# penn-graphics-research/claymore

Hardware: AMD Instinct MI355X
Metric: particles*steps/sec (higher is better)
Workload: dtype f32

## Files before the change

### claymore_amd/csrc/claymore_hip.hip

```cpp
#include <hip/hip_runtime.h>

#include <algorithm>
#include <cmath>
#include <cstdio>
#include <cstdlib>
#include <chrono>
#include <cstring>
#include <string>
#include <vector>

#include "../../include/claymore_amd.h"
#include "mpm_kernels.hpp"
#include "mpm_readout.hpp"

using namespace mpm;

namespace {
constexpr int kHaloWords	 = 128;
constexpr int kStatusBlock = ST_WORDS + kHaloWords + kMaxVelSlots * kMaxVelStride;

struct Partition {
	int* table = nullptr;
	int* keys  = nullptr;
	int* count = nullptr;
// ... 545 lines not shown
	if(ctx->nbc) {
		const int est = std::min(ctx->g.cap, ctx->nbc + ctx->nbc / 16 + 64);
		if(ctx->has_collision)
			grid_update_collision_kernel<<<cdiv(est, 4), 256, 0, s>>>(ctx->g, &ctx->d_status[ST_NBC], ctx->grid[0], ctx->part[ctx->rollid].keys, dt, collision_tick(ctx, dt), ctx->d_maxvel);
		else
			grid_update_kernel<<<cdiv(est, 16), 256, 0, s>>>(ctx->g, &ctx->d_status[ST_NBC], ctx->grid[0], ctx->part[ctx->rollid].keys, dt, ctx->d_maxvel);
	}
	return MPM_OK;
}

int mpm_grid_update(mpm_ctx* ctx, float dt, float* max_vel_sqr) {
	phase_call(ctx);
	if(!ctx || !ctx->ready) return MPM_ERR_NOT_READY;
	HIP_TRY(hipSetDevice(ctx->device));
	hipStream_t s = ctx->s_compute;
	HIP_TRY(hipEventRecord(ctx->ev.start, s));
	int rc = launch_grid_update(ctx, dt);
	if(rc) return rc;
	HIP_TRY(hipEventRecord(ctx->ev.end, s));
	HIP_TRY(hipMemcpyAsync(ctx->h_maxvel, ctx->d_maxvel, sizeof(float) * kMaxVelSlots * kMaxVelStride, hipMemcpyDeviceToHost, s));
	HIP_TRY(hipStreamSynchronize(s));
	HIP_TRY(hipEventElapsedTime(&ctx->timers.grid_update_ms, ctx->ev.start, ctx->ev.end));
	if(max_vel_sqr) *max_vel_sqr = host_maxvel(ctx);
	return MPM_OK;
}

float mpm_compute_dt(const mpm_ctx* ctx, float max_vel, float cur_time, float next_time, float dt_default) {
	float dt = dt_default;
	if(max_vel > 0.0f) dt = std::min(ctx->g.dx * ctx->cfg.cfl / max_vel, dt);
	return std::min(dt, next_time - cur_time);
}

static ModelView make_view(mpm_ctx* ctx, Model& m) {
	const int r = ctx->rollid, n = r ^ 1;
	ModelView v {};
	v.bins_src	 = m.bins[r];
	v.bins_dst	 = m.bins[n];
	v.binoff_src = m.binoff[r];
	v.binoff_dst = m.binoff[n];
	v.list_in	 = m.list[m.list_in];
	v.list_out	 = m.list[m.list_in ^ 1];
	v.size		 = m.size;
	v.row_of	 = m.row_of;
	v.out_count	 = m.out_count;
	v.keep		 = m.keep;
	v.blockinfo	 = m.blockinfo;
	v.pairinfo_in  = m.pairinfo[0];
	v.pairinfo_out = m.pairinfo[1];
	v.mc		 = m.mc;
	return v;
}

static ReadoutArgs make_readout_args(mpm_ctx* ctx, const Model& m) {
	const int r = ctx->rollid;
	return ReadoutArgs {ctx->g, m.nch, m.pair ? 1 : 0, ctx->part[r].keys, ctx->part[r].table, ctx->part[r ^ 1].table, m.size, m.row_of, m.list[m.list_in], m.binoff[r], m.bins[r]};
}

static inline int hint_blocks(const mpm_ctx* ctx, int n) {
	const long long h = (long long) n + n / 16 + 64;
	return (int) ((std::min<long long>(h, std::max(ctx->g.cap, 8)) + 7) & ~7ll);
}

static void launch_g2p2g_model(mpm_ctx* ctx, Model& m, const int* block_list, const int* nblocks_ptr, int nblocks, float dt, float next_dt, hipStream_t s, const int* only_flag = nullptr) {
	const int r = ctx->rollid;
	ModelView v = make_view(ctx, m);
	const int* cur_keys	  = ctx->part[r].keys;
	const GridCfg& g = ctx->g;
	StepConst sk;
	sk.dtp	= dt * g.dx_inv;
	sk.dts	= dt * (4.f * g.dx_inv);
	sk.pred = next_dt * g.dx_inv;
	sk.am	= m.mc.mass * g.dx * g.dx * g.d_inv;
	const float cs = -next_dt * g.d_inv * g.dx;
	sk.ss	= StressScale {2.f * m.mc.mu * m.mc.volume * cs, m.mc.lambda * m.mc.volume * cs, m.mc.volume * cs};
	sk.refl_lim = sk.dts > 0.f ? (1.f / 3.f) / sk.dts : 3.0e38f;
	sk.jdiv		= g.dx * dt * g.d_inv;
	sk.jvisc	= g.dx * g.d_inv * m.mc.viscosity;
	const int nwg = nblocks_ptr ? hint_blocks(ctx, nblocks) : nblocks;
	auto kernel = g2p2g_for<3>(m.pair);
	switch(m.material) {
		case MPM_J_FLUID: kernel = g2p2g_for<0>(m.pair); break;
		case MPM_FIXED_COROTATED: kernel = g2p2g_for<1>(m.pair); break;
		case MPM_SAND: kernel = g2p2g_for<2>(m.pair); break;
		default: break;
	}
	kernel<<<nwg, kG2P2GThreads, 0, s>>>(ctx->g, v, cur_keys, ctx->grid[0], ctx->grid[1], block_list, only_flag, nblocks_ptr, nblocks, dt, next_dt, sk, ctx->d_status);
}

static int launch_clear(mpm_ctx* ctx, int flags) {
	if((flags & kClearRebuild) && !(flags & kClearP2G)) {
		if(ctx->rebuild_cleared) flags &= ~(kClearRebuild | kClearMaxVel);
		ctx->rebuild_cleared = false;
	}
	if(!(flags & (kClearP2G | kClearRebuild))) return MPM_OK;
	ClearArgs a {};
	a.flags	  = flags;
	a.nmodels = (int) ctx->models.size();
	for(int mi = 0; mi < a.nmodels; ++mi) a.out_count[mi] = ctx->models[mi].out_count, a.keep[mi] = ctx->models[mi].keep;
	a.p2g_grid	   = ctx->grid[1];
	a.status	   = ctx->d_status;
	a.max_vel_bits = ctx->d_maxvel;
	Partition& Pn  = ctx->part[ctx->rollid ^ 1];
	a.old_table	   = Pn.table;
	a.old_keys	   = Pn.keys;
	a.old_count	   = Pn.count;
	substep_clear_kernel<<<1024, 256, 0, ctx->s_compute>>>(ctx->g, a);
	return MPM_OK;
}
static int launch_g2p2g_prologue(mpm_ctx* ctx, bool with_rebuild = false, bool fused_update = false) {
	int rc = launch_clear(ctx, with_rebuild ? (kClearP2G | kClearRebuild | (fused_update ? kClearMaxVel : 0)) : kClearP2G);
	if(rc == MPM_OK && with_rebuild) ctx->rebuild_cleared = true;
	return rc;
}

static int launch_g2p2g(mpm_ctx* ctx, float dt, float next_dt, hipEvent_t e0, hipEvent_t e1, bool with_rebuild_clear = false, bool fused_update = false) {
	hipStream_t s = ctx->s_compute;
	int rc		  = launch_g2p2g_prologue(ctx, with_rebuild_clear, fused_update);
	if(rc) return rc;
	HIP_TRY(hipEventRecord(e0, s));
	if(ctx->pbc)
		for(auto& m: ctx->models) launch_g2p2g_model(ctx, m, nullptr, &ctx->d_status[ST_PBC], ctx->pbc, dt, next_dt, s);
	HIP_TRY(hipEventRecord(e1, s));
	return MPM_OK;
}

int mpm_g2p2g(mpm_ctx* ctx, float dt, float next_dt) {
	phase_call(ctx);
	if(!ctx || !ctx->ready) return MPM_ERR_NOT_READY;
	HIP_TRY(hipSetDevice(ctx->device));
	int rc = launch_g2p2g(ctx, dt, next_dt, ctx->ev.g2p2g_start, ctx->ev.g2p2g_end);
	if(rc) return rc;
	HIP_TRY(hipGetLastError());
	HIP_TRY(hipStreamSynchronize(ctx->s_compute));
	HIP_TRY(hipEventElapsedTime(&ctx->last_g2p2g_ms, ctx->ev.g2p2g_start, ctx->ev.g2p2g_end));
	ctx->timers.g2p2g_ms = ctx->last_g2p2g_ms;
	return MPM_OK;
}

static int launch_prepare(mpm_ctx* ctx, int cur, int prev, bool list_is_out, int binoff_sel, const int* pbc_ptr, int nblocks_est, bool sort, bool publish) {
	if(nblocks_est <= 0 && !publish) return MPM_OK;
	PrepareModels pm {};
	pm.n = (int) ctx->models.size();
	for(int mi = 0; mi < pm.n; ++mi) {
		Model& m		  = ctx->models[mi];
		pm.list[mi]		  = m.list[list_is_out ? (m.list_in ^ 1) : m.list_in];
		pm.size[mi]		  = m.size;
		pm.row_of[mi]	  = m.row_of;
		pm.binoff_src[mi] = m.binoff[binoff_sel];
		pm.blockinfo[mi]  = m.blockinfo;
		pm.keep[mi]		  = sort && list_is_out ? m.keep : nullptr;
		pm.pairinfo[mi]	  = m.pair ? m.pairinfo[0] : nullptr;
		pm.pairhand[mi]	  = m.pairinfo[1];
	}
	const int nwg = std::max(1, std::min(ctx->g.cap, nblocks_est + nblocks_est / 16 + 64));
	int* pub	  = publish ? ctx->d_status : nullptr;
	if(sort)
		prepare_blocks_kernel<true><<<nwg, 64, 0, ctx->s_compute>>>(ctx->g, pm, pbc_ptr, ctx->part[cur].table, ctx->part[cur].keys, ctx->part[prev].table, pub, ctx->part[cur].count);
	else
		prepare_blocks_kernel<false><<<nwg, 64, 0, ctx->s_compute>>>(ctx->g, pm, pbc_ptr, ctx->part[cur].table, ctx->part[cur].keys, ctx->part[prev].table, pub, ctx->part[cur].count);
	return MPM_OK;
}

static int launch_rebuild_prepare(mpm_ctx* ctx) {
	const int r = ctx->rollid, n = r ^ 1;
	const int ebc_est = std::min(ctx->g.cap, ctx->ebc + ctx->ebc / 16 + 1024);
	return launch_prepare(ctx, n, r, true, n, &ctx->d_status[ST_CNT_P], ebc_est, true, true);
}
static int launch_rebuild(mpm_ctx* ctx, float fuse_dt = 0.f, bool without_prepare = false) {
	if(fuse_dt == 0.f) fuse_dt = ctx->fuse_dt_once;
	ctx->fuse_dt_once = 0.f;
	hipStream_t s = ctx->s_compute;
	GridCfg& g	  = ctx->g;
	const int r = ctx->rollid, n = r ^ 1;
	Partition& Pn = ctx->part[n];
	Partition& Pr = ctx->part[r];
	const bool fused = fuse_dt > 0.f;
	ctx->grid_momentum = !fused;
	int rc			 = launch_clear(ctx, kClearRebuild | (fused ? kClearMaxVel : 0));
	if(rc) return rc;
	RebuildModels rm {};
	rm.n = (int) ctx->models.size();
	for(int mi = 0; mi < rm.n; ++mi) {
		Model& m		 = ctx->models[mi];
		rm.out_count[mi] = m.out_count;
		rm.size[mi]		 = m.size;
		rm.row_of[mi]	 = m.row_of;
		rm.binoff[mi]	 = m.binoff[r];
		rm.bin_cap[mi]	 = (long long) m.bin_cap;
	}
	int* st			  = ctx->d_status;
	const int ebc_est = std::min(g.cap, ctx->ebc + ctx->ebc / 16 + 1024);
	compact_blocks_kernel<<<std::max(1u, cdiv(ebc_est, 1024)), 1024, 0, s>>>(g, rm, Pr.keys, Pn.keys, Pn.table, st);
	const unsigned rg8 = std::max(1u, std::min(4096u, cdiv((size_t) ebc_est * 8, 256))), rg32 = std::max(1u, std::min(8192u, cdiv((size_t) ebc_est * 32, 256)));
	register_blocks_kernel<0, 1><<<rg8, 256, 0, s>>>(g, &st[ST_CNT_P], nullptr, &st[ST_CNT_N], &st[ST_PBC], Pn.table, Pn.keys, st);
	if(fused) {
		if(ctx->has_collision)
			carry_grid_kernel<true, true><<<2048, 256, 0, s>>>(g, st, Pn.keys, Pr.table, ctx->grid[1], ctx->grid[0], fuse_dt, ctx->d_maxvel, collision_tick(ctx, fuse_dt));
		else
			carry_grid_kernel<true><<<2048, 256, 0, s>>>(g, st, Pn.keys, Pr.table, ctx->grid[1], ctx->grid[0], fuse_dt, ctx->d_maxvel, NoCollision {});
		ctx->grid_preupdated = true;
		ctx->preupdate_dt	 = fuse_dt;
	} else
		carry_grid_kernel<false><<<2048, 256, 0, s>>>(g, st, Pn.keys, Pr.table, ctx->grid[1], ctx->grid[0], 0.f, nullptr, NoCollision {});
	register_blocks_kernel<-1, 1><<<rg32, 256, 0, s>>>(g, &st[ST_CNT_P], &st[ST_CNT_N], &st[ST_CNT_E], &st[ST_NBC], Pn.table, Pn.keys, st);
	if(without_prepare) return MPM_OK;
	return launch_prepare(ctx, n, r, true, n, &st[ST_CNT_P], ebc_est, true, true);
}

static int grow_capacity(mpm_ctx* ctx) {
	if(!ctx->cfg.grow) return MPM_OK;
	hipStream_t s	   = ctx->s_compute;
	const size_t table = (size_t) ctx->g.G * ctx->g.G * ctx->g.G;
	const size_t cap   = (size_t) ctx->g.cap;
	if((size_t) ctx->ebc * 4 > cap * 3 && cap < table) {
		const size_t ncap = std::min(table, cap * 3 / 2 + 1);
		HIP_TRY(hipDeviceSynchronize());
		for(int i = 0; i < 2; ++i) {
			HIP_TRY(regrow(&ctx->part[i].keys, 3 * cap, 3 * ncap, s));
			HIP_TRY(regrow(&ctx->grid[i], cap * 256, ncap * 256, s));
		}
		for(auto& m: ctx->models) {
			for(int i = 0; i < 2; ++i) {
				HIP_TRY(regrow(&m.binoff[i], cap + 1, ncap + 1, s));
				HIP_TRY(regrow(&m.list[i], cap * (size_t) ctx->g.ppb, ncap * (size_t) ctx->g.ppb, s));
			}
			HIP_TRY(regrow(&m.size, cap + 1, ncap + 1, s));
			HIP_TRY(regrow(&m.row_of, cap + 1, ncap + 1, s));
			HIP_TRY(regrow(&m.out_count, cap + 1, ncap + 1, s));
			HIP_TRY(regrow(&m.keep, cap + 1, ncap + 1, s));
			HIP_TRY(regrow(&m.blockinfo, cap * (size_t) kInfoRow, ncap * (size_t) kInfoRow, s));
			if(m.pair)
				for(int i = 0; i < 2; ++i) HIP_TRY(regrow(&m.pairinfo[i], (cap + 1) * (size_t) kPairChunks, (ncap + 1) * (size_t) kPairChunks, s));
		}
		if(ctx->d_overlap) {
			HIP_TRY(regrow(&ctx->d_overlap, cap + 1, ncap + 1, s));
			HIP_TRY(regrow(&ctx->d_halo_list, cap + 1, ncap + 1, s));
			HIP_TRY(regrow(&ctx->d_inner_list, cap + 1, ncap + 1, s));
		}
		for(int p = 0; p < 32; ++p)
			if(ctx->d_send_ids[p]) HIP_TRY(regrow(&ctx->d_send_ids[p], cap + 1, ncap + 1, s));
		ctx->g.cap = (int) ncap;
		ctx->capacity_events++;
	}
	for(auto& m: ctx->models) {
		const size_t need = m.n / kBin + (size_t) ctx->g.cap + 1;
		if((size_t) m.bincount * 4 > m.bin_cap * 3 || need > m.bin_cap) {
			const size_t nb = std::max(need, (size_t) m.bincount * 4 > m.bin_cap * 3 ? m.bin_cap * 3 / 2 + 1 : m.bin_cap);
			HIP_TRY(hipDeviceSynchronize());
			for(int i = 0; i < 2; ++i) HIP_TRY(regrow(&m.bins[i], m.bin_cap * m.nch * kBin, nb * m.nch * kBin, s));
			m.bin_cap = nb;
			ctx->capacity_events++;
		}
	}
	return MPM_OK;
}

static void roll_partition(mpm_ctx* ctx) {
	for(auto& m: ctx->models) m.list_in ^= 1;
	ctx->rollid ^= 1;
}

static int check_books(mpm_ctx* ctx) {
	const long long gone = (long long) ctx->h_status[ST_LOST] + (long long) ctx->h_status[ST_DROPPED] + ctx->books_bias;
	long long added = 0, held = 0;
	for(size_t mi = 0; mi < ctx->models.size(); ++mi) {
		const Model& m = ctx->models[mi];
		added += (long long) m.n;
		held += (long long) m.bucketed;
		if(gone == 0 && (long long) m.bucketed != (long long) m.n)
			return fail(ctx, MPM_ERR_INTERNAL,
						"particle books of model " + std::to_string(mi) + " do not balance: " + std::to_string(m.bucketed) + " bucketed of " + std::to_string(m.n) +
							" added, none counted as lost or dropped");
	}
	if(held + gone != added)
		return fail(ctx, MPM_ERR_INTERNAL,
					"particle books do not balance: " + std::to_string(held) + " bucketed + " + std::to_string(ctx->h_status[ST_LOST]) + " lost + " + std::to_string(ctx->h_status[ST_DROPPED]) +
						" dropped != " + std::to_string(added) + " added");
	return MPM_OK;
}

static int apply_status(mpm_ctx* ctx, mpm_counts* counts);
static int sync_counts(mpm_ctx* ctx, mpm_counts* counts) {
	int rc = read_status(ctx);
	if(rc) return rc;
	return apply_status(ctx, counts);
}
static int apply_status(mpm_ctx* ctx, mpm_counts* counts) {
	int rc = check_status(ctx);
	if(rc) return rc;
	ctx->pbc = ctx->h_status[ST_PBC];
	ctx->nbc = ctx->h_status[ST_NBC];
	ctx->ebc = ctx->h_status[ST_EBC];
	ctx->pbc_prev = ctx->h_status[ST_PBCPREV];
	if(ctx->ebc > ctx->g.cap) return fail(ctx, MPM_ERR_CAPACITY, "Too much exterior blocks: " + std::to_string(ctx->ebc));
	for(size_t mi = 0; mi < ctx->models.size(); ++mi) {
		Model& m	   = ctx->models[mi];
		m.bincount_src = ctx->h_status[ST_BINSPREV + mi];
		m.bincount	   = ctx->h_status[ST_BINS0 + mi];
		m.bucketed	   = ctx->h_status[ST_PART0 + mi];
		if((size_t) m.bincount > m.bin_cap) return fail(ctx, MPM_ERR_CAPACITY, "bin capacity exceeded");
	}
	if(ctx->h_status[ST_NONFINITE]) return fail(ctx, MPM_ERR_NONFINITE, "Maximum velocity is infinity");
	rc = check_books(ctx);
	if(rc) return rc;
	rc = grow_capacity(ctx);
	if(rc) return rc;
	if(counts) return mpm_get_counts(ctx, counts);
// ... 427 lines not shown
```

### claymore_amd/csrc/mpm_kernels.hpp

```cpp
#pragma once
#include <hip/hip_runtime.h>
#include <type_traits>

#include "mpm_device_math.hpp"
#include "mpm_collision.hpp"

namespace mpm {

constexpr int kBin		  = 64;
constexpr int kG2P2GThreads = 64;
constexpr int kMaxModels  = 8;
constexpr int kSortKeys		= 216;
constexpr int kKeyBits		= 8;
constexpr int kStay		  = 13;

enum {
	ST_PBC = 0, ST_NBC = 1, ST_EBC = 2, ST_OVERFLOW = 3, ST_LOST = 4, ST_ARENA = 5, ST_DROPPED = 6, ST_NONFINITE = 7, ST_BINS0 = 8, ST_PART0 = 16,
	 ST_CNT_P = 29, ST_CNT_N = 30, ST_CNT_E = 31, ST_BINSPREV = 32, ST_PBCPREV = 40, ST_WORDS = 64
};

struct GridCfg {
	int G;
	int gbits;
	int ppb;
// ... 154 lines not shown
		const float4 m = g[0];
		float4 p0 = g[16], p1 = g[32], p2 = g[48];
		const float gdt = cfg.gravity * dt;
#define MPM_CELL(c)                                                                 \
	if(m.c > 0.0f) {                                                                \
		const float mass_inv = 1.f / m.c;                                           \
		const float v0		 = wx ? 0.0f : p0.c * mass_inv;                         \
		const float v1		 = (wy ? 0.0f : p1.c * mass_inv) + gdt;                 \
		const float v2		 = wz ? 0.0f : p2.c * mass_inv;                         \
		p0.c				 = v0;                                                  \
		p1.c				 = v1;                                                  \
		p2.c				 = v2;                                                  \
		float q				 = v0 * v0 + v1 * v1 + v2 * v2;                         \
		if(q != q) q = __builtin_inff();  \
		vel_sqr = fmaxf(vel_sqr, q);                                                \
	}
		MPM_CELL(x)
		MPM_CELL(y)
		MPM_CELL(z)
		MPM_CELL(w)
#undef MPM_CELL
		g[16] = p0;
		g[32] = p1;
		g[48] = p2;
	}
#pragma unroll
	for(int off = 32; off > 0; off >>= 1) vel_sqr = fmaxf(vel_sqr, __shfl_xor(vel_sqr, off));
	if((threadIdx.x & 63) == 0 && vel_sqr > 0.f) {
		const unsigned bits = __float_as_uint(vel_sqr);
		unsigned* slot		= max_vel_bits + (blockIdx.x & (kMaxVelSlots - 1)) * kMaxVelStride;
		if(bits > __hip_atomic_load(slot, __ATOMIC_RELAXED, __HIP_MEMORY_SCOPE_AGENT)) atomicMax(slot, bits);
	}
}

struct CollisionArgs {
	CollisionObject obj;
	CollisionPose pose;
};
struct NoCollision {};
MPM_DEV float grid_cell_collision(const GridCfg& cfg, const CollisionArgs& col, int kx, int ky, int kz, int cell, float dt, float4& v) {
#pragma clang fp contract(off)
	const bool wx = kx < cfg.boundary || kx >= cfg.G - cfg.boundary;
	const bool wy = ky < cfg.boundary || ky >= cfg.G - cfg.boundary;
	const bool wz = kz < cfg.boundary || kz >= cfg.G - cfg.boundary;
	const float mass_inv = 1.f / v.x;
	float vel[3];
	vel[0] = wx ? 0.0f : v.y * mass_inv;
	vel[1] = (wy ? 0.0f : v.z * mass_inv) + cfg.gravity * dt;
	vel[2] = wz ? 0.0f : v.w * mass_inv;
	const int node[3] = {kx * 4 + (cell >> 4), ky * 4 + ((cell >> 2) & 3), kz * 4 + (cell & 3)};
	collision_resolve(col.obj, col.pose, node, cfg.dx, cfg.G * 4, (float) cfg.boundary * cfg.dx * 4.f, (float) (cfg.G - cfg.boundary) * 4.f * cfg.dx, vel);
	v.y		= vel[0];
	v.z		= vel[1];
	v.w		= vel[2];
	float q = vel[0] * vel[0] + vel[1] * vel[1] + vel[2] * vel[2];
	q += vel[0] * vel[0];
	q += vel[1] * vel[1];
	q += vel[2] * vel[2];
	if(q != q) q = __builtin_inff();
	return q;
}
__global__ __launch_bounds__(256) void grid_update_collision_kernel(GridCfg cfg, const int* __restrict__ nbc_ptr, float* __restrict__ grid, const int* __restrict__ keys, float dt, CollisionArgs col, unsigned* __restrict__ max_vel_bits) {
	const int cell	  = threadIdx.x & 63;
	const int nblocks = min(*nbc_ptr, cfg.cap);
	float vel_sqr	  = 0.f;
	for(int blockno = (blockIdx.x * 256 + threadIdx.x) >> 6; blockno < nblocks; blockno += gridDim.x * 4) {
		const int kx = keys[3 * blockno], ky = keys[3 * blockno + 1], kz = keys[3 * blockno + 2];
		float* g	 = grid + (size_t) blockno * 256 + cell;
		float4 v	 = {g[0], 0.f, 0.f, 0.f};
		if(v.x > 0.0f) {
			v.y = g[64];
			v.z = g[128];
			v.w = g[192];
			vel_sqr = fmaxf(vel_sqr, grid_cell_collision(cfg, col, kx, ky, kz, cell, dt, v));
			g[64]	= v.y;
			g[128]	= v.z;
			g[192]	= v.w;
		}
	}
#pragma unroll
	for(int off = 32; off > 0; off >>= 1) vel_sqr = fmaxf(vel_sqr, __shfl_xor(vel_sqr, off));
	if((threadIdx.x & 63) == 0 && vel_sqr > 0.f) {
		const unsigned bits = __float_as_uint(vel_sqr);
		unsigned* slot		= max_vel_bits + (blockIdx.x & (kMaxVelSlots - 1)) * kMaxVelStride;
		if(bits > __hip_atomic_load(slot, __ATOMIC_RELAXED, __HIP_MEMORY_SCOPE_AGENT)) atomicMax(slot, bits);
	}
}

__global__ __launch_bounds__(64) void pack_lists_kernel(int ppb, const int* __restrict__ size, const int* __restrict__ row_of, const long long* __restrict__ offset, const int* __restrict__ list, int* __restrict__ packed, int dense, const int* __restrict__ pairinfo, int* __restrict__ packed_info) {
	const int b = blockIdx.x;
	const int n = size[b];
	const int* row = list + (size_t) row_of[b] * ppb;
	for(int i = threadIdx.x; i < n; i += 64) {
		const int chunk = i / kListChunk;
		packed[offset[b] + i] = dense ? row[i] : row[chunk * kListChunk + chunk_slot(chunk_records(n, chunk), i - chunk * kListChunk)];
	}
	if(dense && threadIdx.x < kPairChunks) packed_info[(size_t) b * kPairChunks + threadIdx.x] = pairinfo[(size_t) b * kPairChunks + threadIdx.x];
}
__global__ __launch_bounds__(64) void unpack_lists_kernel(int ppb, const int* __restrict__ size, int* __restrict__ row_of, const long long* __restrict__ offset, int* __restrict__ list, const int* __restrict__ packed, int dense, int* __restrict__ pairinfo, const int* __restrict__ packed_info) {
	const int b = blockIdx.x;
	const int n = size[b];
	int* row	= list + (size_t) b * ppb;
	for(int i = threadIdx.x; i < n; i += 64) {
		const int chunk = i / kListChunk;
		if(dense)
			row[i] = packed[offset[b] + i];
		else
			row[chunk * kListChunk + chunk_slot(chunk_records(n, chunk), i - chunk * kListChunk)] = packed[offset[b] + i];
	}
	if(dense && threadIdx.x < kPairChunks) pairinfo[(size_t) b * kPairChunks + threadIdx.x] = packed_info[(size_t) b * kPairChunks + threadIdx.x];
	if(threadIdx.x == 0) row_of[b] = b;
}
__global__ __launch_bounds__(256) void table_from_keys_kernel(GridCfg cfg, int n, const int* __restrict__ keys, int* __restrict__ table) {
	const int i = blockIdx.x * 256 + threadIdx.x;
	if(i < n) table[key_index(cfg, keys[3 * i], keys[3 * i + 1], keys[3 * i + 2])] = i;
}

__global__ __launch_bounds__(256) void pack_sdf_kernel(size_t n, const float* __restrict__ sd, const float* __restrict__ gx, const float* __restrict__ gy, const float* __restrict__ gz, float4* __restrict__ out) {
	const size_t i = (size_t) blockIdx.x * 256 + threadIdx.x;
	if(i < n) out[i] = make_float4(sd[i], gx[i], gy[i], gz[i]);
}

__device__ __forceinline__ void dir_components(int dir, int& dx, int& dy, int& dz) {
	dz = (dir % 3) - 1;
	dy = ((dir / 3) % 3) - 1;
	dx = (dir / 9) - 1;
}

constexpr int kInfoRow = 64;
struct PrepareModels {
	int n;
	int* list[kMaxModels];
	const int* size[kMaxModels];
	const int* row_of[kMaxModels];
	const int* binoff_src[kMaxModels];
	int* blockinfo[kMaxModels];
	const int* keep[kMaxModels];
	int* pairinfo[kMaxModels];
	const int* pairhand[kMaxModels];
};
template<bool SORT>
__global__ __launch_bounds__(64) void prepare_blocks_kernel(GridCfg cfg, PrepareModels pm, const int* __restrict__ pbc_ptr, const int* __restrict__ cur_table, const int* __restrict__ cur_keys, const int* __restrict__ prev_table, int* __restrict__ publish, int* __restrict__ part_count) {
	constexpr int kPrepChunk = kListChunk;
	__shared__ int s_sorted[kPairChunkMax];
	__shared__ int s_cnt[256];
	__shared__ int s_cur[256];
	const int lane = threadIdx.x;
	if(publish && blockIdx.x == 0 && lane == 0) {
		const int ebc	 = publish[ST_CNT_P] + publish[ST_CNT_N] + publish[ST_CNT_E];
		publish[ST_EBC] = ebc;
		*part_count		 = ebc;
	}
	const int pbc = min(*pbc_ptr, cfg.cap);
	for(int b = blockIdx.x; b < pbc; b += gridDim.x) {
	const int kx = cur_keys[3 * b], ky = cur_keys[3 * b + 1], kz = cur_keys[3 * b + 2];
	int size0 = 0, row0 = 0, keep0 = -2, hand0 = 0;
	if constexpr(SORT) {
		if(pm.n > 0) {
			size0 = pm.size[0][b];
			row0  = pm.row_of[0][b];
			if(pm.keep[0]) keep0 = pm.keep[0][row0];
			if(pm.pairinfo[0]) hand0 = pm.pairhand[0][(size_t) row0 * kPairChunks + (lane & (kPairChunks - 1))];
		}
	}
	int srcno = -1, other = -1;
	if(lane < 27) {
		int ox, oy, oz;
		dir_components(lane, ox, oy, oz);
		srcno = table_query(cfg, prev_table, kx + ox, ky + oy, kz + oz);
	} else if(lane < 54) {
		int ox, oy, oz;
		dir_components(lane - 27, ox, oy, oz);
		other = table_query(cfg, cur_table, kx - ox, ky - oy, kz - oz);
	} else if(lane < 62) {
		const int lb = lane - 54;
		other		 = table_query(cfg, cur_table, kx + ((lb >> 2) & 1), ky + ((lb >> 1) & 1), kz + (lb & 1));
	}
	const int key_shift		= cfg.pid_bits;
	const int tag_shift		= cfg.pid_bits + kKeyBits;
	const unsigned rec_mask = (1u << (tag_shift + 5)) - 1u;
	for(int m = 0; m < pm.n; ++m) {
		int info = other;
		if constexpr(SORT) {
		const int size = __builtin_amdgcn_readfirstlane(m == 0 ? size0 : pm.size[m][b]);
		const int row  = __builtin_amdgcn_readfirstlane(m == 0 ? row0 : pm.row_of[m][b]);
		int* list	   = pm.list[m] + (size_t) row * cfg.ppb;
		const int tail	= size & (kPrepChunk - 1);
		int* pairinfo	= pm.pairinfo[m] ? pm.pairinfo[m] + (size_t) b * kPairChunks : nullptr;
		const int kept	= m == 0 ? keep0 : (pm.keep[m] ? pm.keep[m][row] : -2);
		const bool same = pm.keep[m] && size > 0 && kept == size && (pairinfo || tail <= 64 || (tail & 63) == 0);
		constexpr int NIT = kPrepChunk / 64;
		unsigned recs[NIT];
		auto load_chunk = [&](int chunk0, int nrec) {
#pragma unroll
			for(int it = 0; it < NIT; ++it) recs[it] = (unsigned) list[chunk0 + min(it * 64 + lane, nrec - 1)];
		};
		if(size > 0 && !same) load_chunk(0, min(kPrepChunk, size));
		if(lane < 27) info = srcno >= 0 ? pm.binoff_src[m][srcno] : -1;
		auto sort_chunk = [&](int chunk0, int nrec) {
#pragma unroll
			for(int q = 0; q < 4; ++q) s_cnt[lane + 64 * q] = 0;
			__syncthreads();
			int rank[NIT];
#pragma unroll
			for(int it = 0; it < NIT; ++it) {
				rank[it] = 0;
				if(it * 64 + lane < nrec) rank[it] = atomicAdd(&s_cnt[(recs[it] >> key_shift) & 255], 1);
			}
			__syncthreads();
			{
				const int c0 = s_cnt[4 * lane], c1 = s_cnt[4 * lane + 1], c2 = s_cnt[4 * lane + 2], c3 = s_cnt[4 * lane + 3];
				const int incl = wave_scan_incl(c0 + c1 + c2 + c3);
				const int excl = incl - (c0 + c1 + c2 + c3);
				__syncthreads();
				s_cnt[4 * lane]		= excl;
				s_cnt[4 * lane + 1] = excl + c0;
				s_cnt[4 * lane + 2] = excl + c0 + c1;
				s_cnt[4 * lane + 3] = excl + c0 + c1 + c2;
			}
			__syncthreads();
			const int S = (nrec + 63) >> 6;
			int first[NIT];
#pragma unroll
			for(int it = 0; it < NIT; ++it) first[it] = s_cnt[(recs[it] >> key_shift) & 255];
			__builtin_amdgcn_sched_barrier(0);
#pragma unroll
			for(int it = 0; it < NIT; ++it) {
				if(it * 64 + lane < nrec) {
					const unsigned rec = recs[it] & rec_mask;
					const int p		   = first[it] + rank[it];
					const int pos	   = div_small(p, S);
					s_sorted[(p - pos * S) * 64 + pos] = (int) rec;
				}
			}
			__syncthreads();
			int out[NIT];
#pragma unroll
			for(int it = 0; it < NIT; ++it) out[it] = s_sorted[it * 64 + lane];
			__builtin_amdgcn_sched_barrier(0);
#pragma unroll
			for(int it = 0; it < NIT; ++it)
				if(it < S && lane < slice_records(nrec, it)) list[chunk0 + it * 64 + lane] = out[it];
			__syncthreads();
		};
		auto sort_chunk_pairs = [&](int chunk0, int nrec) {
			const bool big = nrec > kPrepChunk;
			const int n0 = min(nrec, kPrepChunk), n1g = nrec - n0;
#pragma unroll
			for(int q = 0; q < 4; ++q) s_cnt[lane + 64 * q] = 0, s_cur[lane + 64 * q] = 0;
			__syncthreads();
			int rank[NIT];
#pragma unroll
			for(int it = 0; it < NIT; ++it) {
				rank[it] = 0;
				if(it * 64 + lane < n0) rank[it] = atomicAdd(&s_cnt[(recs[it] >> key_shift) & 255], 1);
			}
			if(big) {
#pragma unroll
				for(int it = 0; it < kPairTailMerge / 64; ++it) recs[it] = (unsigned) list[chunk0 + kPrepChunk + min(it * 64 + lane, n1g - 1)];
#pragma unroll
				for(int it = 0; it < kPairTailMerge / 64; ++it)
					if(it * 64 + lane < n1g) atomicAdd(&s_cnt[(recs[it] >> key_shift) & 255], 1);
			}
			__syncthreads();
			int pf;
			{
				int c[4], v[4];
#pragma unroll
				for(int i = 0; i < 4; ++i) {
					c[i] = s_cnt[4 * lane + i];
					v[i] = (c[i] >> 1) | ((c[i] & 1) << 16);
				}
				const int incl = wave_scan_incl(v[0] + v[1] + v[2] + v[3]);
				const int tot  = __builtin_amdgcn_readlane(incl, 63);
				pf			  = tot & 0xffff;
				int excl	  = incl - (v[0] + v[1] + v[2] + v[3]);
#pragma unroll
				for(int i = 0; i < 4; ++i) {
					s_cnt[4 * lane + i] = (excl & 0x3ff) | ((excl >> 16) << 10) | (c[i] << 18);
					excl += v[i];
				}
			}
			__syncthreads();
			const PairChunk pc = pair_chunk(nrec, pf);
			const int n1s	   = pc.L - pc.px;
			auto place = [&](unsigned rec_raw, int r, int e) {
				unsigned rec = rec_raw & rec_mask;
				const int nk = e >> 18, pp = e & 0x3ff;
				int p, member;
				const bool paired = r < (nk & ~1);
				if(paired) {
					p	   = pp + (r >> 1);
					member = r & 1;
				} else {
					const int j = (e >> 10) & 0xff;
					if(j < n1s) {
						p	   = pc.px + j;
						member = 0;
					} else {
						p	   = pc.pf + ((j - n1s) >> 1);
						member = (j - n1s) & 1;
					}
				}
				const int ln = div_small(p, pc.S), d = p - ln * pc.S;
				int pos, ca, cb;
				pair_slice(pc, d, pos, ca, cb);
				int arena = ln & 1;
				if(!paired) {
					int i0 = d - (pp - div_small(pp, pc.S) * pc.S);
					i0 += i0 < 0 ? pc.S : 0;
					if(i0 < (nk >> 1)) arena = 1 ^ (div_small(pp + i0, pc.S) & 1);
				}
				rec |= (unsigned) arena << kArenaBit;
				s_sorted[pos + (member ? ca : 0) + ln] = (int) rec;
			};
			int ent[NIT];
			if(!big) {
#pragma unroll
				for(int it = 0; it < NIT; ++it) ent[it] = s_cnt[(recs[it] >> key_shift) & 255];
				__builtin_amdgcn_sched_barrier(0);
#pragma unroll
				for(int it = 0; it < NIT; ++it)
					if(it * 64 + lane < n0) place(recs[it], rank[it], ent[it]);
			} else {
				auto place_group = [&](int ng) {
#pragma unroll
					for(int it = 0; it < NIT; ++it) {
						if(it * 64 + lane < ng) {
							const int key = (recs[it] >> key_shift) & 255;
							const int r	  = atomicAdd(&s_cur[key], 1);
							place(recs[it], r, s_cnt[key]);
						}
					}
				};
				place_group(n1g);
				load_chunk(chunk0, n0);
				place_group(n0);
			}
			__syncthreads();
			{
				int out[NIT];
#pragma unroll
				for(int it = 0; it < NIT; ++it) out[it] = s_sorted[it * 64 + lane];
				__builtin_amdgcn_sched_barrier(0);
#pragma unroll
				for(int it = 0; it < NIT; ++it)
					if(it * 64 + lane < n0) list[chunk0 + it * 64 + lane] = out[it];
			}
			if(big) {
#pragma unroll
				for(int it = 0; it < kPairTailMerge / 64; ++it)
					if(it * 64 + lane < n1g) list[chunk0 + kPrepChunk + it * 64 + lane] = s_sorted[kPrepChunk + it * 64 + lane];
			}
			if(lane == 0) pairinfo[chunk0 / kPrepChunk] = pf;
			__syncthreads();
		};
		if(pairinfo && same && lane < kPairChunks) pairinfo[lane] = m == 0 ? hand0 : pm.pairhand[m][(size_t) row * kPairChunks + lane];
		for(int chunk0 = 0; chunk0 < size && !same; chunk0 += kPrepChunk) {
			const int left = size - chunk0;
			const int nrec = (pairinfo && left > kPrepChunk && left <= kPairChunkMax) ? left : min(kPrepChunk, left);
			if(chunk0) load_chunk(chunk0, min(kPrepChunk, nrec));
			if(pairinfo)
				sort_chunk_pairs(chunk0, nrec);
			else
				sort_chunk(chunk0, nrec);
			if(nrec > kPrepChunk) break;
		}
		}
		if constexpr(!SORT) {
			if(lane < 27) info = srcno >= 0 ? pm.binoff_src[m][srcno] : -1;
		}
		pm.blockinfo[m][(size_t) b * kInfoRow + lane] = info;
	}
	}
}

}
#include "mpm_g2p2g.hpp"
#include "mpm_g2p2g_pair.hpp"
namespace mpm {

struct RebuildModels {
	int n;
	const int* out_count[kMaxModels];
	int* size[kMaxModels];
	int* row_of[kMaxModels];
	int* binoff[kMaxModels];
	long long bin_cap[kMaxModels];
};

enum { kClearP2G = 1, kClearRebuild = 2, kClearMaxVel = 4 };
struct ClearArgs {
	int flags;
	int nmodels;
	int* out_count[kMaxModels];
	int* keep[kMaxModels];
	float* p2g_grid;
	int* status;
	unsigned* max_vel_bits;
	int* old_table;
	const int* old_keys;
	const int* old_count;
};
__global__ __launch_bounds__(256) void substep_clear_kernel(GridCfg cfg, ClearArgs a) {
	const int tid = blockIdx.x * 256 + threadIdx.x, nthreads = gridDim.x * 256;
	if(a.flags & kClearP2G) {
		const int nbc = min(a.status[ST_NBC], cfg.cap), ebc = min(a.status[ST_EBC], cfg.cap);
		float4* g	  = reinterpret_cast<float4*>(a.p2g_grid);
		for(int i = tid; i < nbc * 64; i += nthreads) g[i] = make_float4(0.f, 0.f, 0.f, 0.f);
		for(int m = 0; m < a.nmodels; ++m)
			for(int i = tid; i <= ebc; i += nthreads) a.out_count[m][i] = 0, a.keep[m][i] = -1;
	}
	if(a.flags & kClearRebuild) {
		const int n = min(*a.old_count, cfg.cap);
		for(int i = tid; i < n; i += nthreads) a.old_table[key_index(cfg, a.old_keys[3 * i], a.old_keys[3 * i + 1], a.old_keys[3 * i + 2])] = -1;
		if(blockIdx.x == gridDim.x - 1) {
			if(threadIdx.x < kMaxModels) {
				a.status[ST_BINSPREV + threadIdx.x] = a.status[ST_BINS0 + threadIdx.x];
				a.status[ST_BINS0 + threadIdx.x]	= 0;
				a.status[ST_PART0 + threadIdx.x]	= 0;
			}
			if(threadIdx.x >= 8 && threadIdx.x < 11) a.status[ST_CNT_P + threadIdx.x - 8] = 0;
			if(threadIdx.x == 11) a.status[ST_PBCPREV] = a.status[ST_PBC];
			if(threadIdx.x >= 64 && threadIdx.x < 64 + kMaxVelSlots) {
				unsigned* slot = a.max_vel_bits + (threadIdx.x - 64) * kMaxVelStride;
				if(*slot >= 0x7f800000u) a.status[ST_NONFINITE] = 1;
				if(a.flags & kClearMaxVel) *slot = 0u;
			}
		}
	}
}

__global__ __launch_bounds__(1024) void compact_blocks_kernel(GridCfg cfg, RebuildModels rm, const int* __restrict__ old_keys, int* __restrict__ new_keys, int* __restrict__ new_table, int* __restrict__ status) {
	__shared__ int s_part[kMaxModels];
	const int ebc = min(status[ST_EBC], cfg.cap);
	for(int b0 = blockIdx.x * blockDim.x; b0 < ebc; b0 += gridDim.x * blockDim.x) {
		const int b = b0 + threadIdx.x;
		int c[kMaxModels];
		bool any = false;
		for(int m = 0; m < rm.n; ++m) {
			c[m] = b < ebc ? rm.out_count[m][b] : 0;
			if(c[m] > cfg.ppb) {
				atomicAdd(&status[ST_DROPPED], c[m] - cfg.ppb);
				c[m] = cfg.ppb;
			}
			any |= c[m] > 0;
		}
		__syncthreads();
		if(threadIdx.x < kMaxModels) s_part[threadIdx.x] = 0;
		__syncthreads();
		for(int m = 0; m < rm.n; ++m) {
			int t = c[m];
#pragma unroll
			for(int off = 32; off > 0; off >>= 1) t += __shfl_xor(t, off);
			if((threadIdx.x & 63) == 0 && t) atomicAdd(&s_part[m], t);
		}
		__syncthreads();
		if((int) threadIdx.x < rm.n && s_part[threadIdx.x]) atomicAdd(&status[ST_PART0 + threadIdx.x], s_part[threadIdx.x]);
		const int nb = block_append(&status[ST_CNT_P], any ? 1 : 0);
		int kx = 0, ky = 0, kz = 0;
		if(any) {
			kx = old_keys[3 * b], ky = old_keys[3 * b + 1], kz = old_keys[3 * b + 2];
			new_keys[3 * nb]					  = kx;
			new_keys[3 * nb + 1]				  = ky;
			new_keys[3 * nb + 2]				  = kz;
			new_table[key_index(cfg, kx, ky, kz)] = nb;
		}
		for(int m = 0; m < rm.n; ++m) {
			const int nbins = any ? (c[m] + kBin - 1) / kBin : 0;
			const int first = block_append(&status[ST_BINS0 + m], nbins);
			if(any) {
				const bool fits = (long long) first + nbins <= rm.bin_cap[m];
				if(!fits) atomicOr(&status[ST_OVERFLOW], 4);
				rm.size[m][nb]	 = fits ? c[m] : 0;
				rm.row_of[m][nb] = b;
				rm.binoff[m][nb] = (nbins && fits) ? first : 0;
			}
		}
	}
}

template<int LO, int HI>
__global__ __launch_bounds__(256) void register_blocks_kernel(GridCfg cfg, const int* __restrict__ pbc_ptr, const int* __restrict__ base2_ptr, int* counter, int* publish, int* table, int* keys, int* status) {
	constexpr int W	   = HI - LO + 1;
	constexpr int NOFF = W * W * W;
	constexpr int LPB  = NOFF <= 8 ? 8 : 32;
	const int pbc	   = min(*pbc_ptr, cfg.cap);
	const int base	   = *pbc_ptr + (base2_ptr ? *base2_ptr : 0);
	if(publish && blockIdx.x == 0 && threadIdx.x == 0) *publish = base;
	const long long total = (long long) pbc * LPB;
	const long long bound = (total + blockDim.x - 1) / blockDim.x * blockDim.x;
	for(long long t = (long long) blockIdx.x * blockDim.x + threadIdx.x; t < bound; t += (long long) gridDim.x * blockDim.x) {
		const int b = (int) (t / LPB), o = (int) (t % LPB);
		bool claim	= false;
		int x = 0, y = 0, z = 0;
		size_t i = 0;
		if(t < total && o < NOFF) {
			x = keys[3 * b] + LO + o / (W * W);
			y = keys[3 * b + 1] + LO + (o / W) % W;
			z = keys[3 * b + 2] + LO + o % W;
			if(key_ok(cfg, x, y, z)) {
				i = key_index(cfg, x, y, z);
				if(table[i] == -1) claim = atomicCAS(&table[i], -1, -2) == -1;
			}
		}
		const int idx = base + block_append(counter, claim ? 1 : 0);
		if(claim) {
			if(idx < cfg.cap) {
				table[i]		  = idx;
				keys[3 * idx]	  = x;
				keys[3 * idx + 1] = y;
				keys[3 * idx + 2] = z;
			} else {
				table[i] = -1;
				atomicOr(&status[ST_OVERFLOW], 1);
			}
		}
	}
}

template<bool UPDATE, bool COLLIDE = false>
__global__ __launch_bounds__(256) void carry_grid_kernel(GridCfg cfg, const int* __restrict__ status, const int* __restrict__ new_keys, const int* __restrict__ old_table, const float* __restrict__ p2g_grid, float* __restrict__ grid, float dt, unsigned* __restrict__ max_vel_bits, std::conditional_t<COLLIDE, CollisionArgs, NoCollision> col) {
	static_assert(UPDATE || !COLLIDE, "the collision object belongs to the grid update");
	const int nbc	  = min(status[ST_CNT_P] + status[ST_CNT_N], cfg.cap);
	const int old_nbc = min(status[ST_NBC], cfg.cap);
// ... 210 lines not shown
```

Baseline: 34.78 billion.

## Process two grid blocks per wavefront in prepare_blocks kernel

Each 64-lane workgroup of prepare_blocks now handles two blocks at once, one per 32-lane half. Each half does the neighbour table queries and blockinfo writes for its own block, and each lane does two queries. The per-chunk sort phase still runs on the full wave, once per half-block, and only for blocks whose particle list changed. Half as many workgroups are launched, which cuts per-block latency for the mostly query-bound work but serialises the two sorts inside one workgroup.

```diff
diff --git a/claymore_amd/csrc/claymore_hip.hip b/claymore_amd/csrc/claymore_hip.hip
--- a/claymore_amd/csrc/claymore_hip.hip
+++ b/claymore_amd/csrc/claymore_hip.hip
@@ -721,7 +721,7 @@
 		pm.pairinfo[mi]	  = m.pair ? m.pairinfo[0] : nullptr;
 		pm.pairhand[mi]	  = m.pairinfo[1];
 	}
-	const int nwg = std::max(1, std::min(ctx->g.cap, nblocks_est + nblocks_est / 16 + 64));
+	const int nwg = std::max(1, (std::min(ctx->g.cap, nblocks_est + nblocks_est / 16 + 64) + 1) / 2);
 	int* pub	  = publish ? ctx->d_status : nullptr;
 	if(sort)
 		prepare_blocks_kernel<true><<<nwg, 64, 0, ctx->s_compute>>>(ctx->g, pm, pbc_ptr, ctx->part[cur].table, ctx->part[cur].keys, ctx->part[prev].table, pub, ctx->part[cur].count);
diff --git a/claymore_amd/csrc/mpm_kernels.hpp b/claymore_amd/csrc/mpm_kernels.hpp
--- a/claymore_amd/csrc/mpm_kernels.hpp
+++ b/claymore_amd/csrc/mpm_kernels.hpp
@@ -330,7 +330,10 @@
 		*part_count		 = ebc;
 	}
 	const int pbc = min(*pbc_ptr, cfg.cap);
-	for(int b = blockIdx.x; b < pbc; b += gridDim.x) {
+	const int half = lane >> 5, j = lane & 31;
+	for(int b0 = 2 * blockIdx.x; b0 < pbc; b0 += 2 * gridDim.x) {
+	const bool live = b0 + half < pbc;
+	const int b		= live ? b0 + half : b0;
 	const int kx = cur_keys[3 * b], ky = cur_keys[3 * b + 1], kz = cur_keys[3 * b + 2];
 	int size0 = 0, row0 = 0, keep0 = -2, hand0 = 0;
 	if constexpr(SORT) {
@@ -338,43 +341,76 @@
 			size0 = pm.size[0][b];
 			row0  = pm.row_of[0][b];
 			if(pm.keep[0]) keep0 = pm.keep[0][row0];
-			if(pm.pairinfo[0]) hand0 = pm.pairhand[0][(size_t) row0 * kPairChunks + (lane & (kPairChunks - 1))];
-		}
-	}
-	int srcno = -1, other = -1;
-	if(lane < 27) {
+			if(pm.pairinfo[0]) hand0 = pm.pairhand[0][(size_t) row0 * kPairChunks + (j & (kPairChunks - 1))];
+		}
+	}
+	int srcno = -1, lo = -1, hi = -1;
+	{
 		int ox, oy, oz;
-		dir_components(lane, ox, oy, oz);
-		srcno = table_query(cfg, prev_table, kx + ox, ky + oy, kz + oz);
-	} else if(lane < 54) {
-		int ox, oy, oz;
-		dir_components(lane - 27, ox, oy, oz);
-		other = table_query(cfg, cur_table, kx - ox, ky - oy, kz - oz);
-	} else if(lane < 62) {
-		const int lb = lane - 54;
-		other		 = table_query(cfg, cur_table, kx + ((lb >> 2) & 1), ky + ((lb >> 1) & 1), kz + (lb & 1));
+		if(j < 27) {
+			dir_components(j, ox, oy, oz);
+			srcno = table_query(cfg, prev_table, kx + ox, ky + oy, kz + oz);
+		} else {
+			dir_components(j - 27, ox, oy, oz);
+			lo = table_query(cfg, cur_table, kx - ox, ky - oy, kz - oz);
+		}
+		if(j < 22) {
+			dir_components(j + 5, ox, oy, oz);
+			hi = table_query(cfg, cur_table, kx - ox, ky - oy, kz - oz);
+		} else if(j < 30) {
+			const int lb = j - 22;
+			hi			 = table_query(cfg, cur_table, kx + ((lb >> 2) & 1), ky + ((lb >> 1) & 1), kz + (lb & 1));
+		}
 	}
 	const int key_shift		= cfg.pid_bits;
 	const int tag_shift		= cfg.pid_bits + kKeyBits;
 	const unsigned rec_mask = (1u << (tag_shift + 5)) - 1u;
+	auto unsettled = [&](int m, int size_h, int row_h, int kept_h) {
+		const int tail_h = size_h & (kPrepChunk - 1);
+		const bool same	 = pm.keep[m] && size_h > 0 && kept_h == size_h && (pm.pairinfo[m] || tail_h <= 64 || (tail_h & 63) == 0);
+		return same ? 0 : size_h;
+	};
+	int sort0 = 0;
 	for(int m = 0; m < pm.n; ++m) {
-		int info = other;
+		int info = lo;
+		if(j < 27) info = srcno >= 0 ? pm.binoff_src[m][srcno] : -1;
 		if constexpr(SORT) {
-		const int size = __builtin_amdgcn_readfirstlane(m == 0 ? size0 : pm.size[m][b]);
-		const int row  = __builtin_amdgcn_readfirstlane(m == 0 ? row0 : pm.row_of[m][b]);
-		int* list	   = pm.list[m] + (size_t) row * cfg.ppb;
-		const int tail	= size & (kPrepChunk - 1);
-		int* pairinfo	= pm.pairinfo[m] ? pm.pairinfo[m] + (size_t) b * kPairChunks : nullptr;
-		const int kept	= m == 0 ? keep0 : (pm.keep[m] ? pm.keep[m][row] : -2);
-		const bool same = pm.keep[m] && size > 0 && kept == size && (pairinfo || tail <= 64 || (tail & 63) == 0);
+			const int size_h = m == 0 ? size0 : pm.size[m][b];
+			const int row_h	 = m == 0 ? row0 : pm.row_of[m][b];
+			const int todo	 = unsettled(m, size_h, row_h, m == 0 ? keep0 : (pm.keep[m] ? pm.keep[m][row_h] : -2));
+			if(m == 0) sort0 = todo;
+			if(pm.pairinfo[m] && size_h > 0 && todo == 0 && live && j < kPairChunks)
+				pm.pairinfo[m][(size_t) b * kPairChunks + j] = m == 0 ? hand0 : pm.pairhand[m][(size_t) row_h * kPairChunks + j];
+		}
+		if(live) {
+			int* row_out	= pm.blockinfo[m] + (size_t) b * kInfoRow;
+			row_out[j]		= info;
+			row_out[32 + j] = hi;
+		}
+	}
+	if constexpr(SORT) {
+	for(int m = 0; m < pm.n; ++m) {
+		int todo_h = sort0, row_h = row0;
+		if(m > 0) {
+			row_h  = pm.row_of[m][b];
+			todo_h = unsettled(m, pm.size[m][b], row_h, pm.keep[m] ? pm.keep[m][row_h] : -2);
+		}
+		const int size_lo = __builtin_amdgcn_readlane(todo_h, 0), size_hi = b0 + 1 < pbc ? __builtin_amdgcn_readlane(todo_h, 32) : 0;
+		const int row_lo = __builtin_amdgcn_readlane(row_h, 0), row_hi = __builtin_amdgcn_readlane(row_h, 32);
+#pragma unroll 1
+		for(int h = 0; h < 2; ++h) {
+		const int size = h ? size_hi : size_lo;
+		const int row  = h ? row_hi : row_lo;
+		if(size <= 0) continue;
+		int* list	  = pm.list[m] + (size_t) row * cfg.ppb;
+		int* pairinfo = pm.pairinfo[m] ? pm.pairinfo[m] + (size_t) (b0 + h) * kPairChunks : nullptr;
 		constexpr int NIT = kPrepChunk / 64;
 		unsigned recs[NIT];
 		auto load_chunk = [&](int chunk0, int nrec) {
 #pragma unroll
 			for(int it = 0; it < NIT; ++it) recs[it] = (unsigned) list[chunk0 + min(it * 64 + lane, nrec - 1)];
 		};
-		if(size > 0 && !same) load_chunk(0, min(kPrepChunk, size));
-		if(lane < 27) info = srcno >= 0 ? pm.binoff_src[m][srcno] : -1;
+		load_chunk(0, min(kPrepChunk, size));
 		auto sort_chunk = [&](int chunk0, int nrec) {
 #pragma unroll
 			for(int q = 0; q < 4; ++q) s_cnt[lane + 64 * q] = 0;
@@ -533,8 +569,7 @@
 			if(lane == 0) pairinfo[chunk0 / kPrepChunk] = pf;
 			__syncthreads();
 		};
-		if(pairinfo && same && lane < kPairChunks) pairinfo[lane] = m == 0 ? hand0 : pm.pairhand[m][(size_t) row * kPairChunks + lane];
-		for(int chunk0 = 0; chunk0 < size && !same; chunk0 += kPrepChunk) {
+		for(int chunk0 = 0; chunk0 < size; chunk0 += kPrepChunk) {
 			const int left = size - chunk0;
 			const int nrec = (pairinfo && left > kPrepChunk && left <= kPairChunkMax) ? left : min(kPrepChunk, left);
 			if(chunk0) load_chunk(chunk0, min(kPrepChunk, nrec));
@@ -545,10 +580,7 @@
 			if(nrec > kPrepChunk) break;
 		}
 		}
-		if constexpr(!SORT) {
-			if(lane < 27) info = srcno >= 0 ? pm.binoff_src[m][srcno] : -1;
-		}
-		pm.blockinfo[m][(size_t) b * kInfoRow + lane] = info;
+	}
 	}
 	}
 }
```

Measured after the change: 35.21 billion (median of 6 runs). 1.01x the previous value.
